# BillyXYB/TransEditor

Measured on AMD Instinct MI355X. Metric: 256x256 images/sec/GPU, G+D fwd+bwd, batch 16; 1/2/4/8-GPU scaling, higher is better.
Workload: dtype f32

## Files before the change

### include/te_hip.h

```cpp
#ifndef TE_HIP_H
#define TE_HIP_H

#include <stdint.h>

#ifdef __cplusplus
extern "C" {
#endif

#define TE_ABI_VERSION 3

#define TE_ERR_NULL -1
#define TE_ERR_SHAPE -2
#define TE_ERR_UNSUPPORTED -3
#define TE_ERR_WORKSPACE -4

typedef void* te_stream_t;

int te_version(void);
const char* te_last_error_string(void);
const char* te_arch(void);

int te_bias_act_f32(float* out, const float* x, const float* b, const float* ref, int act, int grad,
                    float alpha, float scale, int64_t size_x, int64_t step_b, int64_t size_b,
                    te_stream_t stream);
// ... 24 lines not shown
                     int pad_x1, int pad_y0, int pad_y1, te_stream_t stream);


#define TE_CONV_3X3 0
#define TE_CONV_T2 1
#define TE_CONV_S2 2
#define TE_CONV_1X1 3
#define TE_CONV_3X3W 4
#define TE_CONV_3X3W6 5

#define TE_CONV_S2S6 6

#define TE_CONV_T2S6 7

#define TE_CONV_1X1S6 8
#define TE_CONV_KINDS 9

#define TE_PACK_FWD 0
#define TE_PACK_DGRAD 1
#define TE_PACK_SWAP 2
#define TE_PACK_WFWD 3
#define TE_PACK_WDGRAD 4
#define TE_PACK_W6FWD 5
#define TE_PACK_W6DGRAD 6
#define TE_PACK_S6FWD 7
#define TE_PACK_S6SWAP 8
#define TE_PACK_T6FWD 9
#define TE_PACK_T6SWAP 10
#define TE_PACK_P6FWD 11
#define TE_PACK_P6DGRAD 12
#define TE_PACK_KINDS 13

int64_t te_conv_packed_numel(int kind_pack, int Co, int Ci, int ksize);
int te_conv_pack_weights_f32(float* wp, const float* w, float wscale, int kind_pack, int Co, int Ci,
                             int ksize, te_stream_t stream);
int te_conv_pack_weights2_f32(float* wp_a, int kind_a, float* wp_b, int kind_b, const float* w, float wscale, int Co, int Ci,
                              int ksize, te_stream_t stream);

int te_conv_pack_weights_multi_f32(int n, float* const* wp, const float* const* w, const float* wscale, const int* kind_pack,
                                   const int* Co, const int* Ci, const int* ksize, te_stream_t stream);

int te_conv_f32(float* out, const float* in, const float* wp, const float* isc, const float* osc,
                const float* bias, int act, int kind, int B, int K, int M, int H, int W,
                te_stream_t stream);
int te_conv_splitk_count(int kind, int B, int K, int M, int H, int W);
int te_conv_wino_supported(int B, int K, int M, int H, int W);
int te_conv_wino6_supported(int B, int K, int M, int H, int W);
int te_conv_s2s6_supported(int B, int K, int M, int H, int W);
int te_conv_t2s6_supported(int B, int K, int M, int H, int W);
int te_conv_p1s6_supported(int B, int K, int M, int H, int W);
int te_conv_wino6_form(int form);
int te_conv_wino6_tiles_per_block(int n);
int te_conv_s2s6_form(int form);
int te_conv_t2s6_form(int form);
int64_t te_conv_t2s6_ws_floats(int B, int K, int H);
int te_conv_ws_f32(float* out, float* ws, const float* in, const float* wp, const float* isc, const float* osc,
                   const float* bias, int act, int kind, int B, int K, int M, int H, int W, te_stream_t stream);
int te_conv_res_f32(float* out, float* ws, const float* in, const float* wp, const float* isc, const float* osc,
                    const float* bias, const float* res, const float* mask_ref, float mask_gain, int act, int kind, int B,
                    int K, int M, int H, int W, te_stream_t stream);

int te_wgrad_slab_count(int kind, int B, int Co, int Ci, int H, int W);
int te_wgrad_pair_form(int kind, int Co, int Ci, int H, int W);
int te_wgrad_split_supported(int kind, int Co, int Ci, int H, int W);
int te_wgrad_split_bf16(int on);
int te_wgrad_t2_wide(int on);
enum { TE_WG6_FP32 = 0, TE_WG6_3X3 = 1, TE_WG6_3X3_PAIR = 2, TE_WG6_T2_WIDE = 3, TE_WG6_T2 = 4, TE_WG6_T2_MASKED = 5, TE_WG6_1X1 = 6 };
int te_wgrad6_form(int kind, int B, int Co, int Ci, int H, int W, int NB);
int te_wgrad_f32(float* slabs, const float* g, const float* x, int kind, int B, int Co, int Ci, int H,
                 int W, int S, te_stream_t stream);
int te_wgrad_group_plan(int kind, int B, int Co, int Ci, int H, int W, int* NB, int* S);
int te_wgrad_group_f32(float* slabs, const float* g, const float* x, int kind, int B, int Co, int Ci, int H, int W, int S, int NB,
                       te_stream_t stream);

int64_t te_wgrad_reduce_ws_floats(int B, int S, int Co, int Ci, int taps, int want_w, int want_isc, int want_osc);
int te_wgrad_reduce_f32(float* gw, float* gisc, float* gosc, float* ws, const float* slabs, const float* w,
                        float wscale, const float* isc, const float* osc, int B, int S, int Co, int Ci,
                        int taps, te_stream_t stream);

int te_rgb_supported(int M, int K, int HW);
int te_rgb_fwd_f32(float* out, const float* x, const float* w, const float* isc, const float* bias, float wscale, int B,
                   int K, int HW, te_stream_t stream);
int te_rgb_dgrad_f32(float* gx, const float* g, const float* w, const float* isc, float wscale, int B, int K, int HW,
                     te_stream_t stream);
int te_rgb_expand_f32(float* out, const float* x3, const float* w, const float* bias, int act, float wscale, int B, int K,
                      int HW, te_stream_t stream);
int te_rgb_wgrad_slab_count(int B, int K, int HW);
int te_rgb_wgrad_f32(float* slabs, const float* g, const float* x, int B, int K, int HW, int S, te_stream_t stream);
int te_rgb_wgrad_sum_f32(float* slabs, const float* g, const float* x, int B, int K, int HW, int S, te_stream_t stream);

int te_attn_fwd_f32(float* o, float* sim, const float* q, const float* k, const float* v, float scale,
                    int N, int G, int M, int L, int D, te_stream_t stream);
int te_attn_bwd_f32(float* gq, float* gk, float* gv, const float* go, const float* gsim_or_null,
                    const float* q, const float* k, const float* v, const float* sim, float scale, int N,
                    int G, int M, int L, int D, te_stream_t stream);

int te_blur_actgrad_tiles(int in_h, int in_w, int kh, int kw, int pad_x0, int pad_x1, int pad_y0, int pad_y1);
int te_blur_actgrad_f32(float* gx, float* partial, const float* g, const float* ref, const float* k, int64_t major, int in_h,
                        int in_w, int kh, int kw, int pad_x0, int pad_x1, int pad_y0, int pad_y1, float alpha, float scale,
                        te_stream_t stream);
int te_blur_gradact_f32(float* gx, float* partial, const float* g, const float* ref, const float* k, int64_t major, int in_h,
                        int in_w, int kh, int kw, int pad_x0, int pad_x1, int pad_y0, int pad_y1, float alpha, float scale,
                        te_stream_t stream);

int te_upfirdn2d_plan(int64_t major, int in_h, int in_w, int minor, int kh, int kw, int up_x, int up_y, int down_x, int down_y,
                      int pad_x0, int pad_x1, int pad_y0, int pad_y1, int* zgroups, int* tiles);
// ... 162 lines not shown
```

### transeditor_amd/_lib.py

```python
import ctypes as C
import os

import torch

from . import _abi

_HERE = os.path.dirname(os.path.abspath(__file__))
LIB_PATH = os.path.join(_HERE, 'libte_hip.so')
HEADER_PATH = os.path.join(_HERE, '..', 'include', 'te_hip.h')
_lib = _protos = None

CONV_3X3, CONV_T2, CONV_S2, CONV_1X1, CONV_3X3W, CONV_3X3W6, CONV_S2S6, CONV_T2S6, CONV_1X1S6 = 0, 1, 2, 3, 4, 5, 6, 7, 8
(PACK_FWD, PACK_DGRAD, PACK_SWAP, PACK_WFWD, PACK_WDGRAD, PACK_W6FWD, PACK_W6DGRAD, PACK_S6FWD, PACK_S6SWAP, PACK_T6FWD,
 PACK_T6SWAP, PACK_P6FWD, PACK_P6DGRAD) = range(13)


def _header_text():
    if not os.path.exists(HEADER_PATH):
        raise RuntimeError(f'{HEADER_PATH} is missing: the bindings of libte_hip.so are read from it')
    with open(HEADER_PATH) as f:
        return f.read()


def _prototypes():
# ... 221 lines not shown
@_op
def conv_pack2(w, kind_a, kind_b, wscale=1.0):
    w = w.contiguous()
    Co, Ci, ks, _ = w.shape
    wa = torch.empty(lib().te_conv_packed_numel(kind_a, Co, Ci, ks), device=w.device, dtype=w.dtype)
    wb = torch.empty(lib().te_conv_packed_numel(kind_b, Co, Ci, ks), device=w.device, dtype=w.dtype)
    _launch('te_conv_pack_weights2_f32', _ptr(wa), kind_a, _ptr(wb), kind_b, _ptr(w), wscale, Co, Ci, ks)
    return wa, wb


@_op
def conv_pack_multi(jobs):
    n = len(jobs)
    if not n:
        return
    for wp, w, _, _ in jobs:
        if not (w.is_contiguous() and wp.is_contiguous()):
            raise RuntimeError('te_hip: conv_pack_multi needs dense weights and buffers')
    arr = lambda ty, vals: (ty * n)(*vals)
    _launch('te_conv_pack_weights_multi_f32', n, arr(C.c_void_p, [_ptr(j[0]) for j in jobs]), arr(C.c_void_p, [_ptr(j[1]) for j in jobs]),
            arr(C.c_float, [float(j[3]) for j in jobs]), arr(C.c_int, [int(j[2]) for j in jobs]),
            arr(C.c_int, [j[1].shape[0] for j in jobs]), arr(C.c_int, [j[1].shape[1] for j in jobs]),
            arr(C.c_int, [j[1].shape[2] for j in jobs]))


def wino_ok(B, K, M, H, W):
    return bool(lib().te_conv_wino_supported(B, K, M, H, W))


def s2s6_ok(B, K, M, H, W):
    return bool(lib().te_conv_s2s6_supported(B, K, M, H, W))


def t2s6_ok(B, K, M, H, W):
    return bool(lib().te_conv_t2s6_supported(B, K, M, H, W))


def p1s6_ok(B, K, M, H, W):
    return bool(lib().te_conv_p1s6_supported(B, K, M, H, W))


def wino6_form(form=-1):
    return int(lib().te_conv_wino6_form(form))


def wino6_tiles_per_block(n=-1):
    return int(lib().te_conv_wino6_tiles_per_block(n))


def s2s6_form(form=-1):
    return int(lib().te_conv_s2s6_form(form))


def t2s6_form(form=-1):
    return int(lib().te_conv_t2s6_form(form))


def wino6_ok(B, K, M, H, W):
    return bool(lib().te_conv_wino6_supported(B, K, M, H, W))


def conv_out_shape(kind, B, M, H, W):
    if kind in (CONV_T2, CONV_T2S6):
        return (B, M, 2 * H + 1, 2 * W + 1)
    return (B, M, H, W)


@_op
def conv(x, wp, kind, M, H, W, isc=None, osc=None, bias=None, act=0, res=None, mask_ref=None, mask_gain=1.0):
    x = x.contiguous()
    if kind == CONV_1X1S6:
        x = _aligned16(x)
    res = _aligned16(res.contiguous()) if res is not None else None
    mask_ref = _aligned16(mask_ref.contiguous()) if mask_ref is not None else None
    B, K = x.shape[0], x.shape[1]
    out = torch.empty(conv_out_shape(kind, B, M, H, W), device=x.device, dtype=x.dtype)
    if res is not None and tuple(res.shape) != tuple(out.shape):
        raise RuntimeError(f'te_hip: residual {tuple(res.shape)} does not match the convolution output {tuple(out.shape)}')
    if mask_ref is not None and tuple(mask_ref.shape) != tuple(out.shape):
        raise RuntimeError(f'te_hip: mask reference {tuple(mask_ref.shape)} does not match the convolution output {tuple(out.shape)}')
    S = lib().te_conv_splitk_count(kind, B, K, M, H, W)
    if S < 1:
        raise RuntimeError(f'te_conv_splitk_count failed ({S})')
    ws = torch.empty((S,) + tuple(out.shape), device=x.device, dtype=x.dtype) if S > 1 else None
    if kind == CONV_T2S6:
        ws = torch.empty(B * K * H, device=x.device, dtype=x.dtype)
    _launch('te_conv_res_f32', _ptr(out), _ptr(ws), _ptr(x), _ptr(wp), _ptr(isc), _ptr(osc), _ptr(bias), _ptr(res), _ptr(mask_ref),
            mask_gain, act, kind, B, K, M, H, W)
    return out


@_op
def wgrad_slabs(g, x, kind, H, W, group=False):
    g, x = g.contiguous(), x.contiguous()
    B, Co, Ci = g.shape[0], g.shape[1], x.shape[1]
    taps = 1 if kind == CONV_1X1 else 9
    if group:
        nb, sc = C.c_int(0), C.c_int(0)
        _check(lib().te_wgrad_group_plan(kind, B, Co, Ci, H, W, C.byref(nb), C.byref(sc)), 'te_wgrad_group_plan')
        if nb.value > 1:
            slabs = torch.empty(B // nb.value, sc.value, Co, Ci, taps, device=g.device, dtype=g.dtype)
            _launch('te_wgrad_group_f32', _ptr(slabs), _ptr(g), _ptr(x), kind, B, Co, Ci, H, W, sc.value, nb.value)
            return slabs
    S = lib().te_wgrad_slab_count(kind, B, Co, Ci, H, W)
    if S <= 0:
        raise RuntimeError(f'te_wgrad_slab_count failed ({S})')
# ... 1024 lines not shown
```

### transeditor_amd/csrc/s2s6.hip

```cpp
#include "split6_common.h"
#ifdef S2_PROF
#define TE_PROF
#endif
#include "te_prof.h"

namespace {

constexpr int WT = 512, GT = 256, KC = 16, BM = 64;
constexpr int TH = 8, TWO = 16, PH = 4;
constexpr int IR = 2 * PH + 1, IC = 2 * TWO + 1;
constexpr int CI = 18;
constexpr int NTAP = 9;
constexpr int U_SLOTS = 3 * NTAP * 2;
constexpr int TP_PLANE = IR * 2 * 2 * CI * 4;
constexpr int TP_DWORDS = 3 * TP_PLANE;
constexpr int NG = (IC + 3) / 4;
constexpr int N_ITEMS = IR * NG * 8;
constexpr int P_IN = (N_ITEMS + GT - 1) / GT;
constexpr int N_SLOT = P_IN + 16 * P_IN;
constexpr int SLOT0 = NTAP * 6 - N_SLOT;
constexpr int UA_TAPS = 5;

PROF_BUFFER(s2s6, 2048 * 8 * 8)

struct S2Args {
    float* out; const float* in; const u32x4* U; const float* isc; const float* osc; const float* bias; const float* res;
    const float* mref; float mgain; int act;
    int B, K, M, H, W, Hi, Wi, ntiles, mblocks, tiles_x, tiles_y, nt8;
};


template <bool ISC, bool TWOIMG>
__device__ __attribute__((optnone)) void s2s6_body(const S2Args& p) {
    constexpr int NIMG = TWOIMG ? 2 : 1;
    extern __shared__ __attribute__((aligned(16))) unsigned char smem_raw[];
    u32x4* ul = reinterpret_cast<u32x4*>(smem_raw);
    const int tid = threadIdx.x, lane = tid & 63, l31 = lane & 31, half = lane >> 5;
    const int wid = __builtin_amdgcn_readfirstlane(tid >> 6);
    const int grp = wid >> 2, wq = wid & 3, wm = wq >> 1, wrl = wq & 1, gt = tid & (GT - 1);
    unsigned* tl = reinterpret_cast<unsigned*>(smem_raw + U_SLOTS * 1024) + grp * TP_DWORDS;
    const u32x4* tl4 = reinterpret_cast<const u32x4*>(tl);
    int tile, mbq;
    if (!split6_tile(p.ntiles, p.nt8, p.mblocks, tile, mbq)) return;
    const int tx = tile % p.tiles_x, ty = (tile / p.tiles_x) % p.tiles_y, b = tile / (p.tiles_x * p.tiles_y);
    const int x0 = tx * TWO, y0 = ty * TH, yh = y0 + PH * grp;
    const size_t iplane = (size_t)p.Hi * p.Wi, oplane = (size_t)p.H * p.W;
    const float* inb = p.in + (size_t)b * p.K * iplane;
    const float* iscb = ISC ? p.isc + (size_t)b * p.K : nullptr;

    f32x16 acc[NIMG], accl[NIMG];
#pragma unroll
    for (int m = 0; m < NIMG; ++m)
#pragma unroll
        for (int r = 0; r < 16; ++r) { acc[m][r] = 0.f; accl[m][r] = 0.f; }

    unsigned g_off[P_IN];
    int l_off[P_IN];
    bool last_col[P_IN], live[P_IN];
    unsigned q2[P_IN];
#pragma unroll
    for (int i = 0; i < P_IN; ++i) {
        const int e = gt + GT * i;
        live[i] = e < N_ITEMS;
        const int ee = live[i] ? e : 0;
        const int cg = ee % NG, q = (ee / NG) & 7, row = ee / (NG * 8);
        last_col[i] = cg == NG - 1;
        g_off[i] = (unsigned)((2 * q * p.Hi + 2 * yh + row) * p.Wi + 2 * x0 + 4 * cg - (last_col[i] ? 3 : 0));
        l_off[i] = (((row * 2 + (q >> 2)) * 2) * CI + 2 * cg) * 4 + (q & 3);
        q2[i] = 2u * q;
    }
    const int MT = p.M >> 5;
    f32x4 rin[P_IN][2];
    f32x2 rsc[P_IN];
#pragma unroll
    for (int i = 0; i < P_IN; ++i) rsc[i] = f32x2{1.f, 1.f};
    const int nstage = p.K / KC, nimg = NIMG * nstage;
    auto fetch_scales = [&](int s) {
        if (ISC) {
#pragma unroll
            for (int i = 0; i < P_IN; ++i) rsc[i] = *reinterpret_cast<const f32x2u*>(iscb + s * KC + q2[i]);
        }
    };
    auto fetch_item = [&](int i, int s) {
#pragma unroll
        for (int h2 = 0; h2 < 2; ++h2)
            rin[i][h2] = *reinterpret_cast<const f32x4u*>(inb + ((size_t)s * KC + h2) * iplane + g_off[i]);
    };
    auto issue = [&](int s) {
        fetch_scales(s);
#pragma unroll
        for (int i = 0; i < P_IN; ++i) fetch_item(i, s);
    };
    auto issue_u = [&](int uh, int j) {
        const u32x4* us = p.U + (size_t)(TWOIMG ? j >> 1 : j) * 27 * MT * 64;
        const int mb = TWOIMG ? 2 * mbq + (j & 1) : mbq;
        const int ntap = uh ? NTAP - UA_TAPS : UA_TAPS, tap0 = uh ? UA_TAPS : 0, n = ntap * 6;
#pragma unroll
        for (int r = 0; r < 8; ++r) {
            const int jw = wq + 4 * r;
            if (jw >= n) break;
            const int piece = jw / (ntap * 2), rem = jw % (ntap * 2), tap = tap0 + (rem >> 1), mt = rem & 1;
            const int pt = piece * NTAP + tap;
            const u32x4* g = us + ((size_t)pt * MT + 2 * mb + mt) * 64 + (unsigned)lane;
            __builtin_amdgcn_global_load_lds((const __attribute__((address_space(1))) void*)g,
                                             (__attribute__((address_space(3))) void*)(ul + (pt * 2 + mt) * 64), 16, 0, 0);
        }
    };
    unsigned res[P_IN][4][3];
    float te = 0.f, to = 0.f, fe = 0.f, fo = 0.f;
    auto arith = [&](int k) {
        if (k < 0) {
        } else if (k < P_IN) {
#pragma unroll
            for (int h2 = 0; h2 < 2; ++h2) {
                f32x4 v = rin[k][h2];
                if (last_col[k]) v[0] = v[3];
                rin[k][h2] = ISC ? v * rsc[k][h2] : v;
                asm volatile("" : "+v"(rin[k][h2]));
            }
        } else if (k < N_SLOT) {
            const int u = (k - P_IN) >> 2, j = (k - P_IN) & 3, i = u >> 2, c = u & 3;
            float ve = 0.f, vo = 0.f;
            if (j == 0) {
                ve = rin[i][0][c]; vo = rin[i][1][c];
            }
            split6_step4(j, ve, vo, te, to, fe, fo, res[i][c][0], res[i][c][1], res[i][c][2]);
        }
    };
    auto write_res = [&]() {
#pragma unroll
        for (int i = 0; i < P_IN; ++i) {
            if (!live[i]) continue;
#pragma unroll
            for (int c = 0; c < 4; ++c) {
                if (c > 0 && last_col[i]) continue;
#pragma unroll
                for (int pc = 0; pc < 3; ++pc) tl[l_off[i] + (c & 1) * CI * 4 + (c >> 1) * 4 + pc * TP_PLANE] = res[i][c][pc];
            }
        }
    };
    const int rr = l31 >> 4, jj = l31 & 15;
    const int b_chunk = ((2 * (2 * wrl + rr) * 2 + half) * 2) * CI + jj;
    const int a_chunk = wm * 64 + lane;
    bf16x8 av[2][3], bv[2][3];
    auto rd1 = [&](int t, int slot, int q) {
        const int ky = t / 3, kx = t % 3;
        if (q < 3) av[slot][q] = __builtin_bit_cast(bf16x8, ul[a_chunk + (q * NTAP + t) * 128]);
        else bv[slot][q - 3] = __builtin_bit_cast(bf16x8, tl4[b_chunk + ((ky * 2) * 2 + (kx & 1)) * CI + (kx >> 1) + (q - 3) * (TP_PLANE / 4)]);
    };

    issue(0);
    if (grp == 0) { issue_u(0, 0); issue_u(1, 0); }
#pragma unroll
    for (int k = 0; k < N_SLOT; ++k) arith(k);
    write_res();
    if constexpr (!TWOIMG) {
        issue(1);
        if (grp == 0) {
// ... 43 lines not shown
                if (work && grp == 1) split6_wait_vm();
                PROF_T(ta);
                split6_barrier();
                PROF_T(tb);
                if (work && grp == 0) {
                    issue_u(0, cs);
                    split6_wait_vm();
                }
                PROF_T(tc);
                PROF_ACC(pc[3], t0, ta); PROF_ACC(pc[4], ta, tb); PROF_ACC(pc[5], tb, tc);
            }
            PROF_T(t8);
            if (!last) split6_barrier();
            PROF_T(t9);
            PROF_ACC(pc[6], t8, t9);
        }
        PROF_ONLY(if (lane == 0 && blockIdx.x < 2048) {
            unsigned long long* d = te_s2s6_prof_buf + ((size_t)blockIdx.x * 8 + wid) * 8;
            _Pragma("unroll")
            for (int i = 0; i < 6; ++i) d[i] = pc[i];
            d[6] = pc[6] | ((__builtin_amdgcn_s_memrealtime() - rstart) << 40);
            d[7] = ((unsigned long long)nstage << 48) | ((__builtin_readcyclecounter() - pstart) & 0xFFFFFFFFFFFFull);
        })
    } else {
        auto multiply = [&](auto mset_tag, int fs) {
            constexpr int MSET = decltype(mset_tag)::value;
#pragma unroll
            for (int q = 0; q < 6; ++q) rd1(0, 0, q);
            __builtin_amdgcn_s_setprio(1);
#pragma unroll
            for (int t = 0; t < NTAP; ++t) {
                const int slot = t & 1;
                if (t == UA_TAPS - 1) split6_barrier();
                __builtin_amdgcn_sched_barrier(0);
#pragma unroll
                for (int q = 0; q < 6; ++q) {
                    split6_product(q, av[slot], bv[slot], acc[MSET], accl[MSET]);
                    if (t + 1 < NTAP && q < 3) { rd1(t + 1, slot ^ 1, 2 * q); rd1(t + 1, slot ^ 1, 2 * q + 1); }
                    const int k = t * 6 + q;
                    if (MSET == 0) {
                        if (k == 5) fetch_scales(fs);
#pragma unroll
                        for (int i = 0; i < P_IN; ++i)
                            if (k == 6 + 12 * i) fetch_item(i, fs);
                    } else {
                        arith(k - SLOT0);
                    }
                    __builtin_amdgcn_sched_barrier(0);
                }
            }
            __builtin_amdgcn_s_setprio(0);
            split6_barrier();
        };
        auto stage = [&](int ph, bool write) {
            const int cs = (ph + 1) >> 1;
            const bool work = cs >= 1 && cs < nimg;
            if (grp == 1 && work) issue_u(1, cs);
            __builtin_amdgcn_sched_barrier(0);
            if (write) write_res();
            if (grp == 1 && work) split6_wait_vm();
            split6_barrier();
            if (grp == 0 && work) {
                issue_u(0, cs);
                split6_wait_vm();
            }
            split6_barrier();
        };
        split6_wait_vm();
        split6_barrier();
        int ph = 0;
        if (grp == 1) { stage(0, false); ph = 1; }
        for (int s = 0; s < nstage; ++s) {
            const int fs = min(s + 1, nstage - 1);
            multiply(std::integral_constant<int, 0>{}, fs);
            stage(ph + 1, false);
            multiply(std::integral_constant<int, 1>{}, fs);
            if (!(grp == 1 && s == nstage - 1)) stage(ph + 3, true);
            ph += 4;
        }
    }

    const float g_pos = p.act == 3 ? 1.4142135623730951f : 1.f;
#pragma unroll
    for (int m = 0; m < NIMG; ++m) {
        const int mbase = (NIMG * mbq + m) * BM + wm * 32;
        const size_t off0 = ((size_t)b * p.M + mbase) * oplane + (size_t)(yh + 2 * wrl + rr) * p.W + x0 + jj;
        float scv[16], biv[16], resv[16], mrefv[16];
#pragma unroll
        for (int r = 0; r < 16; ++r) {
            const int dm = (r & 3) + 8 * (r >> 2) + 4 * half;
            scv[r] = p.osc ? p.osc[(size_t)b * p.M + mbase + dm] : 1.f;
            biv[r] = p.bias ? p.bias[mbase + dm] : 0.f;
        }
        if (p.res) {
#pragma unroll
            for (int r = 0; r < 16; ++r) resv[r] = p.res[off0 + (size_t)((r & 3) + 8 * (r >> 2) + 4 * half) * oplane];
        }
        if (p.mref) {
#pragma unroll
            for (int r = 0; r < 16; ++r) mrefv[r] = p.mref[off0 + (size_t)((r & 3) + 8 * (r >> 2) + 4 * half) * oplane];
        }
#pragma unroll
        for (int r = 0; r < 16; ++r) {
            const int dm = (r & 3) + 8 * (r >> 2) + 4 * half;
            float v = (acc[m][r] + accl[m][r]) * scv[r] + biv[r];
            if (p.act >= 3) v = (v > 0.f ? v : v * 0.2f) * g_pos;
            if (p.res) v += resv[r];
            if (p.mref) v *= mrefv[r] > 0.f ? p.mgain : 0.2f * p.mgain;
            p.out[off0 + (size_t)dm * oplane] = v;
        }
    }
}

template <bool ISC>
__global__ __launch_bounds__(WT, 2) void s2s6_kernel(const S2Args p) { [[clang::always_inline]] s2s6_body<ISC, false>(p); }
template <bool ISC>
__global__ __launch_bounds__(WT, 2) void s2s6q_kernel(const S2Args p) { [[clang::always_inline]] s2s6_body<ISC, true>(p); }

}

PROF_READBACK(s2s6)

extern "C" int te_conv_s2s6_supported(int B, int K, int M, int H, int W) {
    if (!(B > 0 && K >= 32 && K % KC == 0 && M >= BM && M % BM == 0 && H >= TH && H % TH == 0 && W >= TWO && W % TWO == 0)) return 0;
    return ((int64_t)K * (2 * H + 1) * (2 * W + 1) * 4 < 0x7FFFFFFF && (int64_t)B * (H / TH) * (W / TWO) * (M / BM) < 0x7FFFFFF0) ? 1 : 0;
}

static std::atomic<int> g_s2_form{1};
extern "C" int te_conv_s2s6_form(int form) {
    const int old = g_s2_form.load(std::memory_order_relaxed);
    if (form >= 0 && form <= 2) g_s2_form.store(form, std::memory_order_relaxed);
    return old;
}

int te_s2s6_launch(float* out, const float* in, const float* U, const float* isc, const float* osc, const float* bias, const float* res,
                   const float* mask_ref, float mask_gain, int act, int B, int K, int M, int H, int W, hipStream_t s) {
    TE_REQUIRE(te_conv_s2s6_supported(B, K, M, H, W), TE_ERR_UNSUPPORTED,
               "te_conv_f32(TE_CONV_S2S6): needs K %% 16 == 0 (>= 32), M %% 64 == 0, H %% 8 == 0, W %% 16 == 0 (te_conv_s2s6_supported)");
    TE_REQUIRE((reinterpret_cast<uintptr_t>(U) & 15) == 0 && (reinterpret_cast<uintptr_t>(in) & 3) == 0, TE_ERR_UNSUPPORTED,
               "te_conv_f32(TE_CONV_S2S6): 16-byte aligned packed weights required");
    S2Args a{};
    a.out = out; a.in = in; a.U = reinterpret_cast<const u32x4*>(U); a.isc = isc; a.osc = osc; a.bias = bias; a.res = res;
    a.mref = mask_ref; a.mgain = mask_gain; a.act = act;
    a.B = B; a.K = K; a.M = M; a.H = H; a.W = W; a.Hi = 2 * H + 1; a.Wi = 2 * W + 1;
    a.tiles_x = W / TWO; a.tiles_y = H / TH; a.mblocks = M / BM;
    a.ntiles = B * a.tiles_x * a.tiles_y;
    a.nt8 = te::xcd_banded() ? (int)te::cdiv(a.ntiles, 8) : 0;
    const int64_t blocks = te::cdiv(a.ntiles, 8) * 8 * a.mblocks;
    const size_t lds = (size_t)U_SLOTS * 1024 + 2 * (size_t)TP_DWORDS * 4;
    const int form = g_s2_form.load(std::memory_order_relaxed);
    const int64_t blocks_q = te::cdiv(a.ntiles, 8) * 8 * (M / (2 * BM));
    if (split6_two_image(form, M, blocks_q)) {
        a.mblocks = M / (2 * BM);
        SPLIT6_LAUNCH_ISC(s2s6q_kernel, isc, dim3((unsigned)blocks_q), WT, lds, s, a);
    } else {
        SPLIT6_LAUNCH_ISC(s2s6_kernel, isc, dim3((unsigned)blocks), WT, lds, s, a);
    }
    return te::launch_status("te_conv_f32(TE_CONV_S2S6)");
}
```

### transeditor_amd/csrc/split6_common.h

```cpp
#pragma once
#include "conv_common.h"

typedef short bf16x8 __attribute__((ext_vector_type(8)));
typedef __bf16 bf16x2 __attribute__((ext_vector_type(2)));
typedef float f32x2 __attribute__((ext_vector_type(2)));
typedef float f32x2u __attribute__((ext_vector_type(2), aligned(4)));
typedef float f32x4u __attribute__((ext_vector_type(4), aligned(4)));
typedef unsigned u32x4 __attribute__((ext_vector_type(4)));

__device__ __forceinline__ void split6_barrier() { asm volatile("s_waitcnt lgkmcnt(0)\n\ts_barrier" ::: "memory"); }
__device__ __forceinline__ void split6_wait_vm() { asm volatile("s_waitcnt vmcnt(0)" ::: "memory"); }

__device__ __forceinline__ unsigned split6_piece(float te, float to) {
    const f32x2 t = {te, to};
    return __builtin_bit_cast(unsigned, __builtin_convertvector(t, bf16x2));
}
__device__ __forceinline__ unsigned split6_take(float te, float to, float& fe, float& fo) {
    const unsigned h = split6_piece(te, to);
    fe = __builtin_bit_cast(float, h << 16);
    fo = __builtin_bit_cast(float, h & 0xFFFF0000u);
    return h;
}
__device__ __forceinline__ void split6_pin(float& te, float& to, float& fe, float& fo) { asm volatile("" : "+v"(te), "+v"(to), "+v"(fe), "+v"(fo)); }
template <bool PIN_LOW = true>
// ... 11 lines not shown
        if (PIN_LOW) asm volatile("" : "+v"(l));
    }
    split6_pin(te, to, fe, fo);
}
__device__ __forceinline__ void split6_step3(int j, float ve, float vo, float& te, float& to, float& fe, float& fo, unsigned& h, unsigned& m, unsigned& l) {
    if (j == 0) {
        te = ve; to = vo;
        h = split6_take(te, to, fe, fo);
    } else if (j == 1) {
        te -= fe; to -= fo;
        m = split6_take(te, to, fe, fo);
    } else {
        te -= fe; to -= fo;
        l = split6_piece(te, to);
    }
    split6_pin(te, to, fe, fo);
}

__device__ __forceinline__ void split6_product(int q, const bf16x8 (&a)[3], const bf16x8 (&b)[3], f32x16& big, f32x16& small) {
    constexpr int PA[6] = {1, 0, 2, 0, 1, 0}, PB[6] = {1, 2, 0, 1, 0, 0};
    f32x16& d = q < 5 ? small : big;
    d = __builtin_amdgcn_mfma_f32_32x32x16_bf16(a[PA[q]], b[PB[q]], d, 0, 0, 0);
}

__device__ __forceinline__ bool split6_tile(int ntiles, int nt8, int mblocks, int& tile, int& mb) {
    const int xcd = blockIdx.x & 7, jx = blockIdx.x >> 3;
    const int tq = jx / mblocks;
    mb = jx % mblocks;
    tile = nt8 ? (int)(((int64_t)xcd * ntiles) >> 3) + tq : tq * 8 + xcd;
    return tile < (nt8 ? (int)(((int64_t)(xcd + 1) * ntiles) >> 3) : ntiles);
}

__device__ __forceinline__ bool split6_tile_list(int ntiles, int nt8, int mblocks, int lists, int& tile, int& end, int& step, int& mb) {
    step = nt8 ? 1 : 8;
    if (lists == 0) {
        const bool has = split6_tile(ntiles, nt8, mblocks, tile, mb);
        end = tile + step;
        return has;
    }
    const int xcd = blockIdx.x & 7, jx = blockIdx.x >> 3;
    const int lq = jx / mblocks;
    mb = jx % mblocks;
    const int first = nt8 ? (int)(((int64_t)xcd * ntiles) >> 3) : xcd;
    const int nb = nt8 ? (int)(((int64_t)(xcd + 1) * ntiles) >> 3) - first : (ntiles - xcd + 7) >> 3;
    const int lo = (int)((int64_t)lq * nb / lists), hi = (int)((int64_t)(lq + 1) * nb / lists);
    tile = first + step * lo;
    end = first + step * hi;
    return lo < hi;
}


inline bool split6_two_image(int form_sel, int M, int64_t blocks_q) { return form_sel >= 1 && M % 128 == 0 && (form_sel == 2 || blocks_q >= te::kNumCU); }

template <auto KERNEL, class Args>
inline void split6_launch(dim3 grid, int threads, size_t lds, hipStream_t s, const Args& a) {
    static std::atomic<uint64_t> attr_done{0};
    te::allow_big_lds(attr_done, (const void*)KERNEL, 160 * 1024);
    KERNEL<<<grid, threads, lds, s>>>(a);
}
#define SPLIT6_LAUNCH_ISC(kernel, isc, blocks, threads, lds, s, a) \
    ((isc) ? split6_launch<kernel<true>>(blocks, threads, lds, s, a) : split6_launch<kernel<false>>(blocks, threads, lds, s, a))
```

### transeditor_amd/csrc/wino6.hip

```cpp
#include "split6_common.h"
#include "wino6_schedule.h"
#ifdef W6P_PROF
#define TE_PROF
#endif
#include "te_prof.h"

namespace {

constexpr int WT = 512, KC = 16, TW = 32, NP = TW / 2, BM = 64, TH = 8;
constexpr int U_CHUNKS = 36 * 2 * 64;

struct Wino6Args {
    float* out; const float* in; const u32x4* U; const float* isc; const float* osc; const float* bias; const float* res;
    const float* mref; float mgain; int act;
    int B, K, M, H, W, ntiles, mblocks, tiles_x, tiles_y, nt8;
    int lists;
    int lgpw;
};

constexpr int PH = 4, PR = PH + 2;
constexpr int TP_PLANE = PR * 2 * NP * 4;
constexpr int TP_DWORDS = 12 * TP_PLANE;
constexpr int GT = WT / 2;
constexpr int P_IN = (PR * NP * 8) / GT;
// ... 491 lines not shown
                }
                f32x2 resv[4], mrefv[4];
                if (eres) {
#pragma unroll
                    for (int r = r0; r < r0 + 4; ++r)
                        resv[r - r0] = *reinterpret_cast<const f32x2*>(eres + off0 + (size_t)((r & 3) + 8 * (r >> 2)) * eplane + lo);
                }
                if (emref) {
#pragma unroll
                    for (int r = r0; r < r0 + 4; ++r)
                        mrefv[r - r0] = *reinterpret_cast<const f32x2*>(emref + off0 + (size_t)((r & 3) + 8 * (r >> 2)) * eplane + lo);
                }
#pragma unroll
                for (int r = r0; r < r0 + 4; ++r) {
                    float v0 = acc[m][0][r] + acc[m][1][r] + acc[m][2][r];
                    float v1 = acc[m][1][r] - acc[m][2][r] - acc[m][3][r];
                    const float sc = scv[r - r0], bi = biv[r - r0];
                    v0 = v0 * sc + bi;
                    v1 = v1 * sc + bi;
                    if (eact >= 3) {
                        v0 = (v0 > 0.f ? v0 : v0 * 0.2f) * g_pos;
                        v1 = (v1 > 0.f ? v1 : v1 * 0.2f) * g_pos;
                    }
                    if (eres) { v0 += resv[r - r0][0]; v1 += resv[r - r0][1]; }
                    if (emref) {
                        v0 *= mrefv[r - r0][0] > 0.f ? emgain : 0.2f * emgain;
                        v1 *= mrefv[r - r0][1] > 0.f ? emgain : 0.2f * emgain;
                    }
                    f32x2 v; v[0] = v0; v[1] = v1;
                    *reinterpret_cast<f32x2*>(eout + off0 + (size_t)((r & 3) + 8 * (r >> 2)) * eplane + lo) = v;
                }
            }
        }
        if (!has_next) break;
        tile += tile_step;
#pragma unroll
        for (int m = 0; m < 2; ++m)
#pragma unroll
            for (int c = 0; c < 4; ++c)
#pragma unroll
                for (int r = 0; r < 16; ++r) acc[m][c][r] = 0.f;
    }
}

}

static std::atomic<int> g_w6_form{2};
extern "C" int te_conv_wino6_form(int form) {
    const int old = g_w6_form.load(std::memory_order_relaxed);
    if (form >= 1 && form <= 3) g_w6_form.store(form, std::memory_order_relaxed);
    return old;
}

constexpr int W6_MAX_TPB = 4096;
static std::atomic<int> g_w6_tpb{0};
extern "C" int te_conv_wino6_tiles_per_block(int n) {
    const int old = g_w6_tpb.load(std::memory_order_relaxed);
    if (n >= 0 && n <= W6_MAX_TPB) g_w6_tpb.store(n, std::memory_order_relaxed);
    return old;
}

static int w6_auto_tpb(int nt8c, int mblocks) {
    const int64_t rounds1 = te::cdiv((int64_t)8 * nt8c * mblocks, te::kNumCU);
    for (int n = 4; n >= 2; --n) {
        const int64_t blocks = (int64_t)8 * te::cdiv(nt8c, n) * mblocks;
        if (blocks >= te::kNumCU && te::cdiv(blocks, te::kNumCU) * n <= rounds1) return n;
    }
    return 1;
}

PROF_READBACK(w6p)

extern "C" int te_conv_wino6_supported(int B, int K, int M, int H, int W) {
    if (!(B > 0 && K >= 32 && K % 32 == 0 && M >= BM && M % BM == 0 && H >= TH && H % TH == 0)) return 0;
    const bool wide = W >= TW && W % TW == 0, pair16 = W == 16 && B % 2 == 0;
    if (!wide && !pair16) return 0;
    const int64_t tiles = wide ? (int64_t)B * (H / TH) * (W / TW) : (int64_t)(B / 2) * (H / TH);
    if (!wide && tiles * (M / BM) < te::kNumCU / 2) return 0;
    return ((int64_t)K * H * W * 4 * (wide ? 1 : 2) < 0x7FFFFFFF && tiles * (M / BM) < 0x7FFFFFF0) ? 1 : 0;
}

int te_wino6_launch(float* out, const float* in, const float* U, const float* isc, const float* osc, const float* bias, const float* res,
                    const float* mask_ref, float mask_gain, int act, int B, int K, int M, int H, int W, hipStream_t s) {
    TE_REQUIRE(te_conv_wino6_supported(B, K, M, H, W), TE_ERR_UNSUPPORTED,
               "te_conv_f32(TE_CONV_3X3W6): needs K %% 32 == 0, M %% 64 == 0, W %% 32 == 0 (or W == 16 and an even batch), H %% 8 == 0 (te_conv_wino6_supported)");
    TE_REQUIRE(((reinterpret_cast<uintptr_t>(out) | reinterpret_cast<uintptr_t>(U) | reinterpret_cast<uintptr_t>(res) |
                 reinterpret_cast<uintptr_t>(mask_ref)) & 15) == 0 && (reinterpret_cast<uintptr_t>(in) & 3) == 0, TE_ERR_UNSUPPORTED,
               "te_conv_f32(TE_CONV_3X3W6): 16-byte aligned tensors required");
    Wino6Args a{};
    a.out = out; a.in = in; a.U = reinterpret_cast<const u32x4*>(U); a.isc = isc; a.osc = osc; a.bias = bias; a.res = res;
    a.mref = mask_ref; a.mgain = mask_gain; a.act = act;
    a.B = B; a.K = K; a.M = M; a.H = H; a.W = W;
    a.lgpw = W >= TW ? 4 : 3;
    a.tiles_x = W >= TW ? W / TW : 1; a.tiles_y = H / TH; a.mblocks = M / BM;
    a.ntiles = (W >= TW ? B : B / 2) * a.tiles_x * a.tiles_y;
    a.nt8 = te::xcd_banded() ? (int)te::cdiv(a.ntiles, 8) : 0;
    const int64_t blocks = te::cdiv(a.ntiles, 8) * 8 * a.mblocks;
    const int form = g_w6_form.load(std::memory_order_relaxed);
    const int64_t blocks_q = te::cdiv(a.ntiles, 8) * 8 * (M / (2 * BM));
    if (W >= TW && split6_two_image(form - 1, M, blocks_q)) {
        a.mblocks = M / (2 * BM);
        const int nt8c = (int)te::cdiv(a.ntiles, 8);
        int tpb = g_w6_tpb.load(std::memory_order_relaxed);
        if (tpb == 0) tpb = w6_auto_tpb(nt8c, a.mblocks);
        a.lists = tpb >= 2 ? (int)te::cdiv(nt8c, tpb) : 0;
        const int64_t blocks2 = a.lists ? (int64_t)8 * a.lists * a.mblocks : blocks_q;
        const size_t lds = (size_t)U_CHUNKS * 16 + 2 * (size_t)TP_DWORDS * 4;
        SPLIT6_LAUNCH_ISC(wino6q_kernel, isc, dim3((unsigned)blocks2), WT, lds, s, a);
    } else {
        const size_t lds = (size_t)U_CHUNKS * 16 + 2 * (size_t)TP_DWORDS * 4;
        SPLIT6_LAUNCH_ISC(wino6p_kernel, isc, dim3((unsigned)blocks), WT, lds, s, a);
    }
    return te::launch_status("te_conv_f32(TE_CONV_3X3W6)");
}
```

Baseline: 147.8.

## Make stride-2 split6 kernel persistent over tile lists with cross-tile prefetch

The two-image stride-2 Winograd-like conv kernel now processes a list of tiles per block, as the wino6 kernel already does. It prefetches the next tile's inputs and weights during the current tile's last stage and writes an inline epilogue per tile. The goal is to cut block launch and pipeline fill/drain overhead and to reduce tail imbalance across CUs. The auto tiles-per-block heuristic is moved into a shared header, and the U-weight DMA issue is rewritten with a fixed unrolled pattern. The change adds complexity and register pressure, and depends on the wino6_schedule helpers being correct for this kernel.

```diff
diff --git a/include/te_hip.h b/include/te_hip.h
--- a/include/te_hip.h
+++ b/include/te_hip.h
@@ -100,6 +100,7 @@
 int te_conv_wino6_form(int form);
 int te_conv_wino6_tiles_per_block(int n);
 int te_conv_s2s6_form(int form);
+int te_conv_s2s6_tiles_per_block(int n);
 int te_conv_t2s6_form(int form);
 int64_t te_conv_t2s6_ws_floats(int B, int K, int H);
 int te_conv_ws_f32(float* out, float* ws, const float* in, const float* wp, const float* isc, const float* osc,
diff --git a/transeditor_amd/_lib.py b/transeditor_amd/_lib.py
--- a/transeditor_amd/_lib.py
+++ b/transeditor_amd/_lib.py
@@ -297,6 +297,10 @@
     return int(lib().te_conv_s2s6_form(form))
 
 
+def s2s6_tiles_per_block(n=-1):
+    return int(lib().te_conv_s2s6_tiles_per_block(n))
+
+
 def t2s6_form(form=-1):
     return int(lib().te_conv_t2s6_form(form))
 
diff --git a/transeditor_amd/csrc/s2s6.hip b/transeditor_amd/csrc/s2s6.hip
--- a/transeditor_amd/csrc/s2s6.hip
+++ b/transeditor_amd/csrc/s2s6.hip
@@ -1,4 +1,5 @@
 #include "split6_common.h"
+#include "wino6_schedule.h"
 #ifdef S2_PROF
 #define TE_PROF
 #endif
@@ -27,6 +28,7 @@
     float* out; const float* in; const u32x4* U; const float* isc; const float* osc; const float* bias; const float* res;
     const float* mref; float mgain; int act;
     int B, K, M, H, W, Hi, Wi, ntiles, mblocks, tiles_x, tiles_y, nt8;
+    int lists;
 };
 
 
@@ -40,13 +42,13 @@
     const int grp = wid >> 2, wq = wid & 3, wm = wq >> 1, wrl = wq & 1, gt = tid & (GT - 1);
     unsigned* tl = reinterpret_cast<unsigned*>(smem_raw + U_SLOTS * 1024) + grp * TP_DWORDS;
     const u32x4* tl4 = reinterpret_cast<const u32x4*>(tl);
-    int tile, mbq;
-    if (!split6_tile(p.ntiles, p.nt8, p.mblocks, tile, mbq)) return;
-    const int tx = tile % p.tiles_x, ty = (tile / p.tiles_x) % p.tiles_y, b = tile / (p.tiles_x * p.tiles_y);
-    const int x0 = tx * TWO, y0 = ty * TH, yh = y0 + PH * grp;
-    const size_t iplane = (size_t)p.Hi * p.Wi, oplane = (size_t)p.H * p.W;
-    const float* inb = p.in + (size_t)b * p.K * iplane;
-    const float* iscb = ISC ? p.isc + (size_t)b * p.K : nullptr;
+    int tile, tile_end = 0, tile_step = 0, mbq;
+    if constexpr (TWOIMG) {
+        if (!split6_tile_list(p.ntiles, p.nt8, p.mblocks, p.lists, tile, tile_end, tile_step, mbq)) return;
+    } else {
+        if (!split6_tile(p.ntiles, p.nt8, p.mblocks, tile, mbq)) return;
+    }
+    const size_t iplane = (size_t)p.Hi * p.Wi;
 
     f32x16 acc[NIMG], accl[NIMG];
 #pragma unroll
@@ -54,10 +56,46 @@
 #pragma unroll
         for (int r = 0; r < 16; ++r) { acc[m][r] = 0.f; accl[m][r] = 0.f; }
 
+    typedef const __attribute__((address_space(4))) S2Args* KArgs;
+    auto args = [&]() {
+        if constexpr (TWOIMG) {
+            KArgs k = (KArgs)__builtin_amdgcn_kernarg_segment_ptr();
+            asm volatile("" : "+s"(k));
+            return k;
+        } else {
+            return &p;
+        }
+    };
+    auto group = [&]() {
+        int g = grp;
+        if constexpr (TWOIMG) asm volatile("" : "+s"(g));
+        return g;
+    };
+    auto next_tile_of = [&](int t) { return t + (args()->nt8 ? 1 : 8); };
+    const float* inb;
+    const float* iscb = nullptr;
     unsigned g_off[P_IN];
     int l_off[P_IN];
     bool last_col[P_IN], live[P_IN];
     unsigned q2[P_IN];
+    auto set_tile = [&](int t) {
+        const auto a = args();
+        const int aHi = a->Hi, aWi = a->Wi, atx = a->tiles_x, aty = a->tiles_y, aK = a->K;
+        const int tx = t % atx, ty = (t / atx) % aty, b = t / (atx * aty);
+        const int x0 = tx * TWO, yh = ty * TH + PH * group();
+        inb = a->in + (size_t)b * aK * ((size_t)aHi * aWi);
+        if (ISC) iscb = a->isc + (size_t)b * aK;
+        int gto = gt;
+        if constexpr (TWOIMG) asm volatile("" : "+v"(gto));
+#pragma unroll
+        for (int i = 0; i < P_IN; ++i) {
+            const int e = gto + GT * i;
+            const int ee = e < N_ITEMS ? e : 0;
+            const int cg = ee % NG, q = (ee / NG) & 7, row = ee / (NG * 8);
+            g_off[i] = (unsigned)((2 * q * aHi + 2 * yh + row) * aWi + 2 * x0 + 4 * cg - (cg == NG - 1 ? 3 : 0));
+        }
+    };
+    set_tile(tile);
 #pragma unroll
     for (int i = 0; i < P_IN; ++i) {
         const int e = gt + GT * i;
@@ -65,7 +103,6 @@
         const int ee = live[i] ? e : 0;
         const int cg = ee % NG, q = (ee / NG) & 7, row = ee / (NG * 8);
         last_col[i] = cg == NG - 1;
-        g_off[i] = (unsigned)((2 * q * p.Hi + 2 * yh + row) * p.Wi + 2 * x0 + 4 * cg - (last_col[i] ? 3 : 0));
         l_off[i] = (((row * 2 + (q >> 2)) * 2) * CI + 2 * cg) * 4 + (q & 3);
         q2[i] = 2u * q;
     }
@@ -92,18 +129,38 @@
         for (int i = 0; i < P_IN; ++i) fetch_item(i, s);
     };
     auto issue_u = [&](int uh, int j) {
-        const u32x4* us = p.U + (size_t)(TWOIMG ? j >> 1 : j) * 27 * MT * 64;
-        const int mb = TWOIMG ? 2 * mbq + (j & 1) : mbq;
-        const int ntap = uh ? NTAP - UA_TAPS : UA_TAPS, tap0 = uh ? UA_TAPS : 0, n = ntap * 6;
-#pragma unroll
-        for (int r = 0; r < 8; ++r) {
-            const int jw = wq + 4 * r;
-            if (jw >= n) break;
-            const int piece = jw / (ntap * 2), rem = jw % (ntap * 2), tap = tap0 + (rem >> 1), mt = rem & 1;
-            const int pt = piece * NTAP + tap;
-            const u32x4* g = us + ((size_t)pt * MT + 2 * mb + mt) * 64 + (unsigned)lane;
-            __builtin_amdgcn_global_load_lds((const __attribute__((address_space(1))) void*)g,
-                                             (__attribute__((address_space(3))) void*)(ul + (pt * 2 + mt) * 64), 16, 0, 0);
+        if constexpr (TWOIMG) {
+            int wqo = wq;
+            asm volatile("" : "+s"(wqo));
+            const u32x4* us = p.U + ((size_t)(j >> 1) * 27 * MT + 2 * (2 * mbq + (j & 1))) * 64;
+            auto dma = [&](int piece_tap, int mt) {
+                const u32x4* g = us + (unsigned)(piece_tap * MT + mt) * 64u + (unsigned)lane;
+                __builtin_amdgcn_global_load_lds((const __attribute__((address_space(1))) void*)g,
+                                                 (__attribute__((address_space(3))) void*)(ul + (piece_tap * 2 + mt) * 64), 16, 0, 0);
+            };
+            const int tap = (uh ? UA_TAPS : 0) + wqo;
+#pragma unroll
+            for (int piece = 0; piece < 3; ++piece)
+#pragma unroll
+                for (int mt = 0; mt < 2; ++mt) dma(piece * NTAP + tap, mt);
+            if (!uh) {
+                dma((wqo >> 1) * NTAP + UA_TAPS - 1, wqo & 1);
+                if (wqo < 2) dma(2 * NTAP + UA_TAPS - 1, wqo);
+            }
+        } else {
+            const u32x4* us = p.U + (size_t)j * 27 * MT * 64;
+            const int mb = mbq;
+            const int ntap = uh ? NTAP - UA_TAPS : UA_TAPS, tap0 = uh ? UA_TAPS : 0, n = ntap * 6;
+#pragma unroll
+            for (int r = 0; r < 8; ++r) {
+                const int jw = wq + 4 * r;
+                if (jw >= n) break;
+                const int piece = jw / (ntap * 2), rem = jw % (ntap * 2), tap = tap0 + (rem >> 1), mt = rem & 1;
+                const int pt = piece * NTAP + tap;
+                const u32x4* g = us + ((size_t)pt * MT + 2 * mb + mt) * 64 + (unsigned)lane;
+                __builtin_amdgcn_global_load_lds((const __attribute__((address_space(1))) void*)g,
+                                                 (__attribute__((address_space(3))) void*)(ul + (pt * 2 + mt) * 64), 16, 0, 0);
+            }
         }
     };
     unsigned res[P_IN][4][3];
@@ -253,34 +310,99 @@
             __builtin_amdgcn_s_setprio(0);
             split6_barrier();
         };
-        auto stage = [&](int ph, bool write) {
-            const int cs = (ph + 1) >> 1;
-            const bool work = cs >= 1 && cs < nimg;
-            if (grp == 1 && work) issue_u(1, cs);
+        auto stage = [&](int ph, bool write, bool has_next) {
+            const int cs = wino6_sched::renew_image(ph);
+            const bool work = wino6_sched::renew_work(cs, nimg, has_next);
+            const int ci = cs == nimg ? 0 : cs, g = group();
+            if (g == 1 && work) issue_u(1, ci);
             __builtin_amdgcn_sched_barrier(0);
             if (write) write_res();
-            if (grp == 1 && work) split6_wait_vm();
+            if (g == 1 && work) split6_wait_vm();
             split6_barrier();
-            if (grp == 0 && work) {
-                issue_u(0, cs);
+            if (g == 0 && work) {
+                issue_u(0, ci);
                 split6_wait_vm();
             }
             split6_barrier();
         };
         split6_wait_vm();
         split6_barrier();
-        int ph = 0;
-        if (grp == 1) { stage(0, false); ph = 1; }
-        for (int s = 0; s < nstage; ++s) {
-            const int fs = min(s + 1, nstage - 1);
-            multiply(std::integral_constant<int, 0>{}, fs);
-            stage(ph + 1, false);
-            multiply(std::integral_constant<int, 1>{}, fs);
-            if (!(grp == 1 && s == nstage - 1)) stage(ph + 3, true);
-            ph += 4;
-        }
+        __builtin_assume(nstage >= 2);
+        for (;;) {
+            const bool has_next = next_tile_of(tile) < tile_end;
+            int ph = 0;
+            if (wino6_sched::lead_phase(group())) { stage(0, false, has_next); ph = 1; }
+            for (int s = 0; s < nstage; ++s) {
+                bool next_tile;
+                const int fs = wino6_sched::fetch_stage(s, nstage, has_next, next_tile);
+                if (next_tile) set_tile(next_tile_of(tile));
+                multiply(std::integral_constant<int, 0>{}, fs);
+                stage(ph + 1, false, has_next);
+                multiply(std::integral_constant<int, 1>{}, fs);
+                if (wino6_sched::runs_sb(group(), s, nstage, has_next)) stage(ph + 3, true, has_next);
+                ph += 4;
+            }
+            for (int i = 0; i < wino6_sched::tail_barriers(group(), has_next); ++i) split6_barrier();
+
+            const KArgs e = args();
+            const int tx = tile % e->tiles_x, ty = (tile / e->tiles_x) % e->tiles_y, b = tile / (e->tiles_x * e->tiles_y);
+            int elane = lane;
+            asm volatile("" : "+v"(elane));
+            const int ehalf = elane >> 5, err = (elane & 31) >> 4, ejj = elane & 15;
+            int ewq = wq;
+            asm volatile("" : "+s"(ewq));
+            const int ewm = ewq >> 1, ewrl = ewq & 1;
+            const int eM = e->M, eW = e->W, eact = e->act;
+            const size_t eplane = (size_t)e->H * eW;
+            const float emgain = e->mgain;
+            const float g_pos = eact == 3 ? 1.4142135623730951f : 1.f;
+            float* const eout = e->out;
+            const float* const eosc = e->osc; const float* const ebias = e->bias; const float* const eres = e->res; const float* const emref = e->mref;
+#pragma unroll
+            for (int m = 0; m < NIMG; ++m) {
+                const int mbase = (NIMG * mbq + m) * BM + ewm * 32;
+                const size_t off0 = ((size_t)b * eM + mbase) * eplane + (size_t)(ty * TH + PH * group() + 2 * ewrl) * eW + tx * TWO;
+                const unsigned lo = (unsigned)(err * eW + ejj) + 4u * (unsigned)ehalf * (unsigned)eplane;
+#pragma unroll
+                for (int r0 = 0; r0 < 16; r0 += 4) {
+                    float scv[4], biv[4], resv[4], mrefv[4];
+#pragma unroll
+                    for (int r = r0; r < r0 + 4; ++r) {
+                        const int mm = mbase + (r & 3) + 8 * (r >> 2) + 4 * ehalf;
+                        scv[r - r0] = eosc ? eosc[(size_t)b * eM + mm] : 1.f;
+                        biv[r - r0] = ebias ? ebias[mm] : 0.f;
+                    }
+                    if (eres) {
+#pragma unroll
+                        for (int r = r0; r < r0 + 4; ++r) resv[r - r0] = eres[off0 + (size_t)((r & 3) + 8 * (r >> 2)) * eplane + lo];
+                    }
+                    if (emref) {
+#pragma unroll
+                        for (int r = r0; r < r0 + 4; ++r) mrefv[r - r0] = emref[off0 + (size_t)((r & 3) + 8 * (r >> 2)) * eplane + lo];
+                    }
+#pragma unroll
+                    for (int r = r0; r < r0 + 4; ++r) {
+                        float v = (acc[m][r] + accl[m][r]) * scv[r - r0] + biv[r - r0];
+                        if (eact >= 3) v = (v > 0.f ? v : v * 0.2f) * g_pos;
+                        if (eres) v += resv[r - r0];
+                        if (emref) v *= mrefv[r - r0] > 0.f ? emgain : 0.2f * emgain;
+                        eout[off0 + (size_t)((r & 3) + 8 * (r >> 2)) * eplane + lo] = v;
+                    }
+                }
+            }
+            if (!has_next) break;
+            tile = next_tile_of(tile);
+#pragma unroll
+            for (int m = 0; m < NIMG; ++m)
+#pragma unroll
+                for (int r = 0; r < 16; ++r) { acc[m][r] = 0.f; accl[m][r] = 0.f; }
+        }
+        return;
     }
 
+    const int tx = tile % p.tiles_x, ty = (tile / p.tiles_x) % p.tiles_y, b = tile / (p.tiles_x * p.tiles_y);
+    const int x0 = tx * TWO, yh = ty * TH + PH * grp;
+    const size_t oplane = (size_t)p.H * p.W;
     const float g_pos = p.act == 3 ? 1.4142135623730951f : 1.f;
 #pragma unroll
     for (int m = 0; m < NIMG; ++m) {
@@ -331,6 +453,13 @@
 extern "C" int te_conv_s2s6_form(int form) {
     const int old = g_s2_form.load(std::memory_order_relaxed);
     if (form >= 0 && form <= 2) g_s2_form.store(form, std::memory_order_relaxed);
+    return old;
+}
+
+static std::atomic<int> g_s2_tpb{0};
+extern "C" int te_conv_s2s6_tiles_per_block(int n) {
+    const int old = g_s2_tpb.load(std::memory_order_relaxed);
+    if (n >= 0 && n <= SPLIT6_MAX_TPB) g_s2_tpb.store(n, std::memory_order_relaxed);
     return old;
 }
 
@@ -353,7 +482,12 @@
     const int64_t blocks_q = te::cdiv(a.ntiles, 8) * 8 * (M / (2 * BM));
     if (split6_two_image(form, M, blocks_q)) {
         a.mblocks = M / (2 * BM);
-        SPLIT6_LAUNCH_ISC(s2s6q_kernel, isc, dim3((unsigned)blocks_q), WT, lds, s, a);
+        const int nt8c = (int)te::cdiv(a.ntiles, 8);
+        int tpb = g_s2_tpb.load(std::memory_order_relaxed);
+        if (tpb == 0) tpb = split6_auto_tpb(nt8c, a.mblocks);
+        a.lists = tpb >= 2 ? (int)te::cdiv(nt8c, tpb) : 0;
+        const int64_t blocks2 = a.lists ? (int64_t)8 * a.lists * a.mblocks : blocks_q;
+        SPLIT6_LAUNCH_ISC(s2s6q_kernel, isc, dim3((unsigned)blocks2), WT, lds, s, a);
     } else {
         SPLIT6_LAUNCH_ISC(s2s6_kernel, isc, dim3((unsigned)blocks), WT, lds, s, a);
     }
diff --git a/transeditor_amd/csrc/split6_common.h b/transeditor_amd/csrc/split6_common.h
--- a/transeditor_amd/csrc/split6_common.h
+++ b/transeditor_amd/csrc/split6_common.h
@@ -87,6 +87,16 @@
 
 inline bool split6_two_image(int form_sel, int M, int64_t blocks_q) { return form_sel >= 1 && M % 128 == 0 && (form_sel == 2 || blocks_q >= te::kNumCU); }
 
+constexpr int SPLIT6_MAX_TPB = 4096;
+inline int split6_auto_tpb(int nt8c, int mblocks) {
+    const int64_t rounds1 = te::cdiv((int64_t)8 * nt8c * mblocks, te::kNumCU);
+    for (int n = 4; n >= 2; --n) {
+        const int64_t blocks = (int64_t)8 * te::cdiv(nt8c, n) * mblocks;
+        if (blocks >= te::kNumCU && te::cdiv(blocks, te::kNumCU) * n <= rounds1) return n;
+    }
+    return 1;
+}
+
 template <auto KERNEL, class Args>
 inline void split6_launch(dim3 grid, int threads, size_t lds, hipStream_t s, const Args& a) {
     static std::atomic<uint64_t> attr_done{0};
diff --git a/transeditor_amd/csrc/wino6.hip b/transeditor_amd/csrc/wino6.hip
--- a/transeditor_amd/csrc/wino6.hip
+++ b/transeditor_amd/csrc/wino6.hip
@@ -567,22 +567,13 @@
     return old;
 }
 
-constexpr int W6_MAX_TPB = 4096;
 static std::atomic<int> g_w6_tpb{0};
 extern "C" int te_conv_wino6_tiles_per_block(int n) {
     const int old = g_w6_tpb.load(std::memory_order_relaxed);
-    if (n >= 0 && n <= W6_MAX_TPB) g_w6_tpb.store(n, std::memory_order_relaxed);
+    if (n >= 0 && n <= SPLIT6_MAX_TPB)g_w6_tpb.store(n, std::memory_order_relaxed);
     return old;
 }
 
-static int w6_auto_tpb(int nt8c, int mblocks) {
-    const int64_t rounds1 = te::cdiv((int64_t)8 * nt8c * mblocks, te::kNumCU);
-    for (int n = 4; n >= 2; --n) {
-        const int64_t blocks = (int64_t)8 * te::cdiv(nt8c, n) * mblocks;
-        if (blocks >= te::kNumCU && te::cdiv(blocks, te::kNumCU) * n <= rounds1) return n;
-    }
-    return 1;
-}
 
 PROF_READBACK(w6p)
 
@@ -617,7 +608,7 @@
         a.mblocks = M / (2 * BM);
         const int nt8c = (int)te::cdiv(a.ntiles, 8);
         int tpb = g_w6_tpb.load(std::memory_order_relaxed);
-        if (tpb == 0) tpb = w6_auto_tpb(nt8c, a.mblocks);
+        if (tpb == 0) tpb = split6_auto_tpb(nt8c, a.mblocks);
         a.lists = tpb >= 2 ? (int)te::cdiv(nt8c, tpb) : 0;
         const int64_t blocks2 = a.lists ? (int64_t)8 * a.lists * a.mblocks : blocks_q;
         const size_t lds = (size_t)U_CHUNKS * 16 + 2 * (size_t)TP_DWORDS * 4;
```

Result: no change. 148.6 (median of 6 runs) (+0.5%).
